# MingruiYuan/SpoofSV

Measured on AMD Instinct MI355X. Metric: mel-frames/sec (Text2Mel+SSRN train), higher is better.
Workload: dtype f32 (conv GEMMs: fp32 operands scaled by a power of two and split into fp16 hi+lo = 22 significand bits, three exact fp16 MFMAs per product, fp32 accumulate: ~2^-22 per product, gradients within 3e-6 of float64 = the exact-fp32 path's level); 1 GPU; train_text2mel + train_ssrn (train/ordinary.py step: fwd, l1+bin-div+guided-att losses, bwd, Adam), batch 32 utterances/GPU, N=186, T=325, 80 mel -> 513x1300 linear, hidden 256, random-init; global_batch=32, parallelism=dp1, launch=hipGraph replay, ddp=none

## Files before the change

### spoofsv_amd/csrc/api.hip

```cpp
#include <stdarg.h>
#include <stdio.h>
#include <stdlib.h>
#include <string.h>
#include "ssv_common.h"

static thread_local char g_err[512] = "";
int ssv_fail(int code, const char* fmt, ...) {
  va_list ap;
  va_start(ap, fmt);
  vsnprintf(g_err, sizeof(g_err), fmt, ap);
  va_end(ap);
  return code;
}
int ssv_check_launch(const char* what) {
  hipError_t e = hipGetLastError();
  if (e == hipSuccess) return 0;
  ssv_fail(0, "%s: launch failed: %s", what, hipGetErrorString(e));
  return -(int)e;
}
static int g_precision = -1;
static int precision_from_env() {
  const char* e = getenv("SSV_PRECISION");
  if (!e || !*e || !strcmp(e, "f16x2") || !strcmp(e, "2")) return 2;
  if (!strcmp(e, "fp32") || !strcmp(e, "0")) return 0;
  if (!strcmp(e, "bf16x3") || !strcmp(e, "1")) return 1;
  return -1;
}
int ssv_precision() {
  if (g_precision < 0) {
    g_precision = precision_from_env();
    if (g_precision < 0) {
      fprintf(stderr, "libssv_hip: SSV_PRECISION=%s is not one of fp32|0, bf16x3|1, f16x2|2 (call ssv_set_precision to choose a mode)\n", getenv("SSV_PRECISION"));
      abort();
    }
  }
  return g_precision;
}
static const char* const g_knob_names[SSV_T_COUNT] = {"SSV_NT_FORCE", "SSV_NNB_FORCE", "SSV_LN_GROUPS", "SSV_LN_PERSIST", "SSV_LSTM_MERGE", "SSV_PWLN_BWD"};
static char g_knob_val[SSV_T_COUNT][512];
static const char* g_knob[SSV_T_COUNT];
static int g_knobs_loaded = 0;
static void load_knobs() {
  for (int i = 0; i < SSV_T_COUNT; ++i) {
    const char* e = getenv(g_knob_names[i]);
    if (e) { strncpy(g_knob_val[i], e, sizeof g_knob_val[i] - 1); g_knob_val[i][sizeof g_knob_val[i] - 1] = 0; g_knob[i] = g_knob_val[i]; }
    else g_knob[i] = nullptr;
  }
  __atomic_store_n(&g_knobs_loaded, 1, __ATOMIC_RELEASE);
}
const char* ssv_tuning(int knob) {
  if (!__atomic_load_n(&g_knobs_loaded, __ATOMIC_ACQUIRE)) load_knobs();
  return g_knob[knob];
}
extern "C" void ssv_reload_tuning(void) { load_knobs(); }
#include <mutex>
#include <string>
#include <map>
static int g_shape_log = -1;
static std::string g_shape_path;
static std::mutex g_shape_mu;
static std::map<std::string, long>* g_shape_seen = nullptr;
static void shape_log_flush() {
  std::lock_guard<std::mutex> lk(g_shape_mu);
  if (!g_shape_seen) return;
  if (g_shape_path.empty()) return;
  if (FILE* f = fopen(g_shape_path.c_str(), "w")) {
    for (const auto& kv : *g_shape_seen) fprintf(f, "%s\t%ld\n", kv.first.c_str(), kv.second);
    fclose(f);
  }
}
bool ssv_shape_log_on() {
  if (g_shape_log < 0) { const char* e = getenv("SSV_SHAPE_LOG"); g_shape_log = (e && *e) ? 1 : 0; if (g_shape_log) { g_shape_path = e; atexit(shape_log_flush); } }
  return g_shape_log == 1;
}
void ssv_shape_log(const char* kernel, dim3 grid, dim3 block, double flops, double bytes, const char* note) {
  if (!ssv_shape_log_on()) return;
  char line[768];
  snprintf(line, sizeof line, "%s\t%ux%ux%u\t%.6g\t%.6g\t%s", kernel, grid.x * block.x, grid.y * block.y, grid.z * block.z, flops, bytes, note ? note : "");
  std::lock_guard<std::mutex> lk(g_shape_mu);
  if (!g_shape_seen) g_shape_seen = new std::map<std::string, long>();
  ++(*g_shape_seen)[line];
}
extern "C" int ssv_set_precision(int mode) {
  int prev = g_precision >= 0 ? g_precision : precision_from_env();
  if (prev < 0) prev = ssv_fail(SSV_UNSUPPORTED, "SSV_PRECISION=%s is not one of fp32|0, bf16x3|1, f16x2|2; mode %d set explicitly", getenv("SSV_PRECISION"), mode);
  g_precision = mode <= 0 ? 0 : (mode == 1 ? 1 : 2);
  return prev;
}
extern "C" int ssv_get_precision(void) {
  if (g_precision < 0 && precision_from_env() < 0)
    return ssv_fail(SSV_UNSUPPORTED, "SSV_PRECISION=%s is not one of fp32|0, bf16x3|1, f16x2|2", getenv("SSV_PRECISION"));
  return ssv_precision();
}
extern "C" int ssv_version(void) { return 7; }
extern "C" const char* ssv_arch(void) { return "gfx950"; }
extern "C" const char* ssv_last_error(void) { return g_err; }
```

### spoofsv_amd/csrc/api_norm.hip

```cpp
#include "ssv_host.h"

extern "C" size_t ssv_channel_ln_act_fwd_workspace(int B, int C, int L) { (void)B; (void)C; (void)L; return 256; }
extern "C" int ssv_channel_ln_act_fwd(const float* x, long x_bs, const float* gamma, const float* beta, float* y, long y_bs, float* y_amax, float* stats,
                                      int B, int C, int L, int act, void* ws, size_t ws_bytes, ssv_stream_t stream) {
  SSV_CHECK(x && gamma && beta && y && B > 0 && C > 0 && L > 0 && act >= 0 && act <= 2, SSV_BAD_SHAPE, "channel_ln_act_fwd: bad argument");
  SSV_CHECK(B <= 65535, SSV_UNSUPPORTED, "channel_ln_act_fwd: batch %d exceeds grid.y", B);
  (void)ws; (void)ws_bytes;
  return ssv_launch_ln_act_fwd(x, x_bs, gamma, beta, y, y_bs, stats, B, C, L, act, (hipStream_t)stream, y_amax);
}
static size_t ln_part_bytes(int B, int C, int L, int rows_per_block) { return align256((size_t)ssv_ln_gate_bwd_nblk(B, L) * rows_per_block * C * sizeof(float)); }
extern "C" size_t ssv_channel_ln_act_bwd_workspace(int B, int C, int L) { return ln_part_bytes(B, C, L, 3); }
extern "C" int ssv_channel_ln_act_bwd(const float* dy, long dy_bs, const float* x, long x_bs, const float* stats, const float* gamma, const float* beta,
                                      float* dx, long dx_bs, float* pgrads, int B, int C, int L, int act, void* ws, size_t ws_bytes, ssv_stream_t stream) {
  SSV_CHECK(dy && x && stats && gamma && beta && dx && B > 0 && C > 0 && L > 0 && act >= 0 && act <= 2, SSV_BAD_SHAPE, "channel_ln_act_bwd: bad argument");
  SSV_CHECK(ws && ws_bytes >= ssv_channel_ln_act_bwd_workspace(B, C, L), SSV_BAD_SHAPE, "channel_ln_act_bwd: workspace too small");
  return ssv_launch_ln_act_bwd(dy, dy_bs, x, x_bs, stats, gamma, beta, dx, dx_bs, (float*)ws, pgrads, B, C, L, act, (hipStream_t)stream);
}

static bool pwln_fused(int B, int Cin, int Cout, int L) { return use_bf3(B, L, Cin, Cout) && Cout <= 640 && B <= 65535; }
extern "C" size_t ssv_pointwise_conv_ln_act_fwd_workspace(int Cin, int Cout) { return conv_fwd_ws(Cin, Cout, 1).total; }
extern "C" int ssv_pointwise_conv_ln_act_fwd(const float* x, long x_bs, const float* x_amax, int x_namax, const float* w, const void* w_packed, const float* bias,
                                             const float* s, const float* gamma, const float* beta, float* pre, float* stats, float* y, long y_bs, float* y_amax,
                                             int B, int Cin, int Cout, int L, int act, void* ws, size_t ws_bytes, ssv_stream_t stream) {
  SSV_CHECK(x && w && gamma && beta && pre && y && B > 0 && Cin > 0 && Cout > 0 && L > 0 && act >= 0 && act <= 2, SSV_BAD_SHAPE, "pointwise_conv_ln_act_fwd: bad argument");
  SSV_CHECK(x_bs >= (long)Cin * L && y_bs >= (long)Cout * L, SSV_BAD_SHAPE, "pointwise_conv_ln_act_fwd: batch stride smaller than C*L");
  if (pwln_fused(B, Cin, Cout, L) && y_bs == (long)Cout * L && (!y_amax || ssv_amax_rows_(L) >= ssv_cdiv(L, 64))) {
    const ConvWs l = conv_fwd_ws(Cin, Cout, 1);
    SSV_CHECK((w_packed && !(use_f16() && !x_amax)) || (ws && ws_bytes >= l.total), SSV_BAD_SHAPE, "pointwise_conv_ln_act_fwd: workspace too small");
    int shift[3] = {0, 0, 0};
    PwLnArgs pw = {gamma, beta, y, y_bs, stats, y_amax, ssv_amax_rows_(L), act};
    return conv_nn(x, x_bs, w, packed_planes(w_packed, Cout, Cin, 1).fwd, (long)Cin, 1, bias, s, nullptr, 0, pre, (long)Cout * L, B, Cin, Cout, L, 1, shift, true,
                   ws, l, (hipStream_t)stream, x_amax, x_namax, nullptr, &pw);
  }
  SSV_TRY(ssv_conv1d_fwd(x, x_bs, x_amax, x_namax, w, w_packed, bias, s, pre, (long)Cout * L, nullptr, B, Cin, Cout, L, 1, 1, 0, ws, ws_bytes, stream));
  return ssv_channel_ln_act_fwd(pre, (long)Cout * L, gamma, beta, y, y_bs, y_amax, stats, B, Cout, L, act, nullptr, 0, stream);
}

static inline bool hw_colstats(int B, int C, int L) { return use_bf3(B, L, C, 2 * C) && C % 64 == 0 && C <= 512; }
struct HwFwdWs { ConvWs conv; size_t colstats, total; };
static HwFwdWs hw_fwd_ws(int B, int C, int L, int k) {
  HwFwdWs l;
  l.conv = conv_fwd_ws(C, 2 * C, k);
  WsTake t;
  t.take(l.conv.total);
  l.colstats = t.take(hw_colstats(B, C, L) ? (size_t)B * (2 * C / 64) * L * 2 * sizeof(float) : 0);
  l.total = t.off;
  return l;
}
extern "C" size_t ssv_highway_conv1d_fwd_workspace(int B, int C, int L, int k) { return hw_fwd_ws(B, C, L, k).total; }
extern "C" int ssv_highway_conv1d_fwd(const float* x, long x_bs, const float* x_amax, int x_namax, const float* w, const void* w_packed, const float* bias,
                                      const float* g1, const float* b1, const float* g2, const float* b2, float* h, float* stats, float* y, long y_bs,
                                      float* y_amax, int B, int C, int L, int k, int dilation, int causal, void* ws, size_t ws_bytes, ssv_stream_t stream) {
  SSV_CHECK(x && w && g1 && b1 && g2 && b2 && h && y, SSV_BAD_SHAPE, "highway_conv1d_fwd: null argument");
  SSV_CHECK(B > 0 && C > 0 && L > 0 && B <= 65535, SSV_BAD_SHAPE, "highway_conv1d_fwd: bad shape B=%d C=%d L=%d", B, C, L);
  if (hw_colstats(B, C, L)) {
    const HwFwdWs l = hw_fwd_ws(B, C, L, k);
    SSV_CHECK(ws && ws_bytes >= l.total, SSV_BAD_SHAPE, "highway_conv1d_fwd: workspace too small");
    SSV_CHECK(x_bs >= (long)C * L && y_bs >= (long)C * L, SSV_BAD_SHAPE, "highway_conv1d_fwd: batch stride smaller than C*L");
    float* cs = ws_f32(ws, l.colstats);
    int shift[3];
    SSV_TRY(conv_shifts(k, dilation, causal, shift));
    SSV_TRY(conv_nn(x, x_bs, w, packed_planes(w_packed, 2 * C, C, k).fwd, (long)C * k, k, bias, nullptr, nullptr, 0, h, (long)2 * C * L, B, C, 2 * C, L, k, shift, true,
                    ws, l.conv, (hipStream_t)stream, x_amax, x_namax, cs));
    return ssv_launch_ln_gate_fwd_stream(h, x, x_bs, cs, g1, b1, g2, b2, y, y_bs, stats, y_amax, B, C, L, (hipStream_t)stream);
  }
  SSV_TRY(ssv_conv1d_fwd(x, x_bs, x_amax, x_namax, w, w_packed, bias, nullptr, h, (long)2 * C * L, nullptr, B, C, 2 * C, L, k, dilation, causal, ws, ws_bytes, stream));
  return ssv_launch_ln_gate_fwd(h, (long)2 * C * L, x, x_bs, g1, b1, g2, b2, y, y_bs, stats, B, C, L, (hipStream_t)stream, y_amax);
}

static int pw_bwd_ln_and_data(const float* dy, long dy_bs, const float* w, const void* w_packed, const float* gamma, const float* beta, const float* pre,
                              const float* stats, float* dx, long dx_bs, float* dpre, float* dpre_amax, float* part, int B, int Cin, int Cout, int L, int act,
                              void* ws, size_t ws_bytes, ssv_stream_t stream) {
  const long pbs = (long)Cout * L;
  if (dx && w_packed && use_bf3(B, L, Cout, Cin) && (!use_f16() || dpre_amax) && ssv_pwln_bwd_fused_ok(B, Cin, Cout, L)) {
    const bool has_amax = dpre_amax != nullptr;
    const SplitPlanes pl = packed_planes(w_packed, Cout, Cin, 1).tr;
    PwLnBw q;
    q.dy = dy; q.dy_bs = dy_bs; q.pre = pre; q.stats = stats; q.gamma = gamma; q.beta = beta;
    q.dpre = dpre; q.part = part; q.part_rows = ssv_ln_act_bwd_rows(1, Cout, L, has_amax); q.part_q = 4 / ssv_ln_act_bwd_vec(Cout, L, has_amax);
    q.amax = dpre_amax; q.namax = ssv_amax_rows_(L);
    q.Ahi = pl.hi; q.Alo = pl.lo; q.a_inv = pl.inv;
    q.dx = dx; q.dx_bs = dx_bs;
    q.xrow_w = (Cin > 128 && Cin % 128 == 1) ? w + (Cin - 1) : nullptr; q.xrow_sk = Cin;
    q.M = Cout; q.Cin = Cin; q.L = L; q.act = act;
    return ssv_launch_pwln_bwd(q, B, use_f16() ? 1 : 0, (hipStream_t)stream);
  }
  SSV_TRY(ssv_launch_ln_act_bwd(dy, dy_bs, pre, pbs, stats, gamma, beta, dpre, pbs, part, nullptr, B, Cout, L, act, (hipStream_t)stream, dpre_amax));
  if (dx) SSV_TRY(ssv_conv1d_bwd_data(dpre, pbs, dpre_amax, ssv_amax_rows_(L), w, w_packed, nullptr, dx, dx_bs, B, Cin, Cout, L, 1, 1, 0, ws, ws_bytes, stream));
  return 0;
}
struct LinkBwdWs { size_t dpre, part, amax, data, data_bytes, wgrad, wgrad_bytes, total; };
static LinkBwdWs link_bwd_ws(int B, int Cin, int Cout, int L, int k) {
  WsTake t;
  LinkBwdWs l;
  l.dpre = t.take((size_t)B * Cout * L * sizeof(float));
  l.part = t.take(ln_part_bytes(B, Cout, L, 3));
  l.amax = t.take((size_t)B * ssv_amax_rows_(L) * sizeof(float));
  l.data_bytes = ssv_conv1d_bwd_data_workspace(Cin, Cout, k);
  l.data = t.take(l.data_bytes);
  l.wgrad_bytes = ssv_conv1d_bwd_weight_workspace(B, Cin, Cout, L, k);
  l.wgrad = t.take(l.wgrad_bytes);
  l.total = t.off;
  return l;
}
static LinkBwdWs pw_ws(int B, int Cin, int Cout, int L) { return link_bwd_ws(B, Cin, Cout, L, 1); }
static LinkBwdWs hw_ws(int B, int C, int L, int k) { return link_bwd_ws(B, C, 2 * C, L, k); }
extern "C" size_t ssv_pointwise_conv_ln_act_bwd_workspace(int B, int Cin, int Cout, int L) { return pw_ws(B, Cin, Cout, L).total; }
extern "C" int ssv_pointwise_conv_ln_act_bwd(const float* dy, long dy_bs, const float* x, long x_bs, const float* x_amax, int x_namax, const float* w,
                                             const void* w_packed, const float* gamma,
                                             const float* beta, const float* pre, const float* stats, float* dx, long dx_bs, float* dw, float* pgrads,
                                             float* ds, int B, int Cin, int Cout, int L, int act, void* ws, size_t ws_bytes, ssv_stream_t stream) {
  SSV_CHECK(dy && x && w && gamma && beta && pre && stats && dw && pgrads, SSV_BAD_SHAPE, "pointwise_conv_ln_act_bwd: null argument");
  SSV_CHECK(B > 0 && B <= 65535 && Cin > 0 && Cout > 0 && L > 0 && act >= 0 && act <= 2, SSV_BAD_SHAPE, "pointwise_conv_ln_act_bwd: bad shape");
  const LinkBwdWs s = pw_ws(B, Cin, Cout, L);
  SSV_CHECK(ws && ws_bytes >= s.total, SSV_BAD_SHAPE, "pointwise_conv_ln_act_bwd: workspace too small (%zu < %zu)", ws_bytes, s.total);
  float* dpre = ws_f32(ws, s.dpre);
  const long pbs = (long)Cout * L;
  float* da = use_f16() ? ws_f32(ws, s.amax) : nullptr;
  const int dn = ssv_amax_rows_(L);
  SSV_TRY(pw_bwd_ln_and_data(dy, dy_bs, w, w_packed, gamma, beta, pre, stats, dx, dx_bs, dpre, da, ws_f32(ws, s.part), B, Cin, Cout, L, act,
                             ws_f32(ws, s.data), s.data_bytes, stream));
  if (ds) SSV_TRY(ssv_rowsum(dpre, pbs, ds, B, Cout, L, stream));
  return conv1d_bwd_weight_impl(dpre, pbs, x, x_bs, dw, B, Cin, Cout, L, 1, 1, 0, ws_f32(ws, s.wgrad), s.wgrad_bytes, stream,
                                ws_f32(ws, s.part), pgrads, 3 * Cout, ssv_ln_act_bwd_rows(B, Cout, L, da != nullptr), da, dn, x_amax, x_namax);
}

extern "C" size_t ssv_channel_ln_bwd2_workspace(int B, int C, int L) { return ln_part_bytes(B, C, L, 1); }
extern "C" int ssv_channel_ln_bwd2(const float* v, long v_bs, const float* gn, long gn_bs, const float* x, long x_bs, const float* stats,
                                   const float* gamma, float* d_gn, long dgn_bs, float* d_x, long dx_bs, float* dgamma,
                                   int B, int C, int L, void* ws, size_t ws_bytes, ssv_stream_t stream) {
  SSV_CHECK(v && gn && x && stats && gamma && d_gn && d_x && dgamma && B > 0 && B <= 65535 && C > 0 && L > 0, SSV_BAD_SHAPE, "channel_ln_bwd2: bad argument");
  SSV_CHECK(ws && ws_bytes >= ssv_channel_ln_bwd2_workspace(B, C, L), SSV_BAD_SHAPE, "channel_ln_bwd2: workspace too small");
  return ssv_launch_ln_bwd2(v, v_bs, gn, gn_bs, x, x_bs, stats, gamma, d_gn, dgn_bs, d_x, dx_bs, (float*)ws, dgamma, B, C, L, (hipStream_t)stream);
}
extern "C" int ssv_highway_gate_fwd(const float* h, const float* x, long x_bs, const float* g1, const float* b1, const float* g2, const float* b2,
                                    float* stats, float* y, long y_bs, float* y_amax, int B, int C, int L, ssv_stream_t stream) {
  SSV_CHECK(h && x && g1 && b1 && g2 && b2 && y && B > 0 && B <= 65535 && C > 0 && L > 0, SSV_BAD_SHAPE, "highway_gate_fwd: bad argument");
  return ssv_launch_ln_gate_fwd(h, (long)2 * C * L, x, x_bs, g1, b1, g2, b2, y, y_bs, stats, B, C, L, (hipStream_t)stream, y_amax);
}
extern "C" size_t ssv_highway_gate_bwd2_workspace(int B, int C, int L) { return ln_part_bytes(B, C, L, 4); }
extern "C" int ssv_highway_gate_bwd2(const float* vh, const float* vx, long vx_bs, const float* gy, long gy_bs, const float* h, const float* x, long x_bs,
                                     const float* stats, const float* g1, const float* b1, const float* g2, const float* b2,
                                     float* d_gy, long dgy_bs, float* d_h, float* d_x, long dx_bs, float* pgrads,
                                     int B, int C, int L, void* ws, size_t ws_bytes, ssv_stream_t stream) {
  SSV_CHECK(vh && vx && gy && h && x && stats && g1 && b1 && g2 && b2 && d_gy && d_h && d_x && pgrads && B > 0 && B <= 65535 && C > 0 && L > 0,
            SSV_BAD_SHAPE, "highway_gate_bwd2: bad argument");
  SSV_CHECK(ws && ws_bytes >= ssv_highway_gate_bwd2_workspace(B, C, L), SSV_BAD_SHAPE, "highway_gate_bwd2: workspace too small");
  return ssv_launch_ln_gate_bwd2(vh, vx, vx_bs, gy, gy_bs, h, x, x_bs, stats, g1, b1, g2, b2, d_gy, dgy_bs, d_h, d_x, dx_bs, (float*)ws, pgrads,
                                 B, C, L, (hipStream_t)stream);
}

extern "C" size_t ssv_highway_gate_bwd_workspace(int B, int C, int L) { return ln_part_bytes(B, C, L, 6); }
extern "C" int ssv_highway_gate_bwd(const float* dy, long dy_bs, const float* x, long x_bs, const float* g1, const float* b1,
                                    const float* g2, const float* b2, const float* h, const float* stats, float* dh, float* dxres,
                                    long dx_bs, float* pgrads, int B, int C, int L, void* ws, size_t ws_bytes, ssv_stream_t stream) {
  SSV_CHECK(dy && x && g1 && b1 && g2 && b2 && h && stats && dh && dxres && B > 0 && C > 0 && L > 0 && B <= 65535, SSV_BAD_SHAPE, "highway_gate_bwd: bad argument");
  SSV_CHECK(ws && ws_bytes >= ssv_highway_gate_bwd_workspace(B, C, L), SSV_BAD_SHAPE, "highway_gate_bwd: workspace too small");
  return ssv_launch_ln_gate_bwd(dy, dy_bs, h, x, x_bs, stats, g1, b1, g2, b2, dh, dxres, dx_bs, (float*)ws, pgrads, B, C, L, (hipStream_t)stream);
}

extern "C" size_t ssv_highway_conv1d_bwd_workspace(int B, int C, int L, int k) { return hw_ws(B, C, L, k).total; }
extern "C" int ssv_highway_conv1d_bwd(const float* dy, long dy_bs, const float* x, long x_bs, const float* x_amax, int x_namax, const float* w, const void* w_packed,
                                      const float* g1, const float* b1,
                                      const float* g2, const float* b2, const float* h, const float* stats, float* dx, long dx_bs, float* dw,
                                      float* pgrads, int B, int C, int L, int k, int dilation, int causal, void* ws, size_t ws_bytes,
                                      ssv_stream_t stream) {
  SSV_CHECK(dy && x && w && g1 && b1 && g2 && b2 && h && stats && dx && dw && pgrads, SSV_BAD_SHAPE, "highway_conv1d_bwd: null argument");
  SSV_CHECK(B > 0 && C > 0 && L > 0 && B <= 65535, SSV_BAD_SHAPE, "highway_conv1d_bwd: bad shape B=%d C=%d L=%d", B, C, L);
  const LinkBwdWs s = hw_ws(B, C, L, k);
  SSV_CHECK(ws && ws_bytes >= s.total, SSV_BAD_SHAPE, "highway_conv1d_bwd: workspace too small (%zu < %zu)", ws_bytes, s.total);
  float* dH = ws_f32(ws, s.dpre);
  float* da = use_f16() ? ws_f32(ws, s.amax) : nullptr;
  const int dn = ssv_amax_rows_(L);
  SSV_TRY(ssv_launch_ln_gate_bwd(dy, dy_bs, h, x, x_bs, stats, g1, b1, g2, b2, dH, dx, dx_bs, ws_f32(ws, s.part), nullptr, B, C, L, (hipStream_t)stream, da));
  SSV_TRY(ssv_conv1d_bwd_data(dH, (long)2 * C * L, da, dn, w, w_packed, dx, dx, dx_bs, B, C, 2 * C, L, k, dilation, causal, ws_f32(ws, s.data), s.data_bytes, stream));
  return conv1d_bwd_weight_impl(dH, (long)2 * C * L, x, x_bs, dw, B, C, 2 * C, L, k, dilation, causal, ws_f32(ws, s.wgrad), s.wgrad_bytes, stream,
                                ws_f32(ws, s.part), pgrads, 6 * C, ssv_ln_gate_bwd_rows(B, C, L, da != nullptr), da, dn, x_amax, x_namax);
}

extern "C" int ssv_ln_partial_rows(int B, int L) { return ssv_ln_gate_bwd_nblk(B, L); }
extern "C" int ssv_ln_bwd_partial_rows(int gate, int B, int C, int L, int with_amax) {
  return gate ? ssv_ln_gate_bwd_rows(B, C, L, with_amax != 0) : ssv_ln_act_bwd_rows(B, C, L, with_amax != 0);
}
extern "C" size_t ssv_highway_conv1d_bwd_data_workspace(int B, int C, int L, int k) { (void)B; (void)L; return ssv_conv1d_bwd_data_workspace(C, 2 * C, k); }
extern "C" int ssv_highway_conv1d_bwd_data(const float* dy, long dy_bs, const float* x, long x_bs, const float* w, const void* w_packed,
                                           const float* g1, const float* b1, const float* g2, const float* b2, const float* h, const float* stats,
                                           float* dx, long dx_bs, float* dh, float* dh_amax, float* part, int B, int C, int L, int k, int dilation, int causal,
                                           void* ws, size_t ws_bytes, ssv_stream_t stream) {
  SSV_CHECK(dy && x && w && g1 && b1 && g2 && b2 && h && stats && dx && dh && part, SSV_BAD_SHAPE, "highway_conv1d_bwd_data: null argument");
  SSV_CHECK(B > 0 && C > 0 && L > 0 && B <= 65535, SSV_BAD_SHAPE, "highway_conv1d_bwd_data: bad shape B=%d C=%d L=%d", B, C, L);
  SSV_TRY(ssv_launch_ln_gate_bwd(dy, dy_bs, h, x, x_bs, stats, g1, b1, g2, b2, dh, dx, dx_bs, part, nullptr, B, C, L, (hipStream_t)stream, dh_amax));
  return ssv_conv1d_bwd_data(dh, (long)2 * C * L, dh_amax, ssv_amax_rows_(L), w, w_packed, dx, dx, dx_bs, B, C, 2 * C, L, k, dilation, causal, ws, ws_bytes, stream);
}
extern "C" size_t ssv_pointwise_conv_ln_act_bwd_data_workspace(int B, int Cin, int Cout, int L) { (void)B; (void)L; return ssv_conv1d_bwd_data_workspace(Cin, Cout, 1); }
extern "C" int ssv_pointwise_conv_ln_act_bwd_data(const float* dy, long dy_bs, const float* w, const void* w_packed, const float* gamma, const float* beta,
                                                  const float* pre, const float* stats, float* dx, long dx_bs, float* ds, float* dpre, float* dpre_amax,
                                                  float* part, int B, int Cin, int Cout, int L, int act, void* ws, size_t ws_bytes, ssv_stream_t stream) {
  SSV_CHECK(dy && w && gamma && beta && pre && stats && dpre && part, SSV_BAD_SHAPE, "pointwise_conv_ln_act_bwd_data: null argument");
  SSV_CHECK(B > 0 && B <= 65535 && Cin > 0 && Cout > 0 && L > 0 && act >= 0 && act <= 2, SSV_BAD_SHAPE, "pointwise_conv_ln_act_bwd_data: bad shape");
  const long pbs = (long)Cout * L;
  SSV_TRY(pw_bwd_ln_and_data(dy, dy_bs, w, w_packed, gamma, beta, pre, stats, dx, dx_bs, dpre, dpre_amax, part, B, Cin, Cout, L, act, ws, ws_bytes, stream));
  if (ds) SSV_TRY(ssv_rowsum(dpre, pbs, ds, B, Cout, L, stream));
  return 0;
}
```

### spoofsv_amd/csrc/bf3_tuning.h

```cpp
#pragma once

#ifndef SSV_NN_XONE
#define SSV_NN_XONE 1
#endif

#define SSV_NN_XBUF(KT, WM, NT) (!((KT) == 3 && (NT) == 6))

#ifndef SSV_NN_HALO_SMALL
#define SSV_NN_HALO_SMALL 16
#endif

#define SSV_NNB_WAVES(KT, WM, NT, EPI, HW) \
  (((KT) == 1 && (WM) == 2 && (NT) == 4 && (EPI) == 0) || ((KT) == 3 && (WM) == 2 && (NT) == 7 && (EPI) == 0 && (HW) == 16) ? 3 : 2)

#ifndef SSV_NNBW_XROW
#define SSV_NNBW_XROW 1
#endif

#ifndef SSV_NNBW_PARK
#define SSV_NNBW_PARK 1
#endif

#ifndef SSV_NT_RING
#define SSV_NT_RING 1
#endif

#ifndef SSV_NT_XROW
#define SSV_NT_XROW 1
#endif

#ifndef SSV_PWLN_XROW
#define SSV_PWLN_XROW 1
#endif

#ifndef SSV_PWLN_ROLL
#define SSV_PWLN_ROLL 1
#endif

#ifndef SSV_PWLN_PARK
#define SSV_PWLN_PARK 1
#endif

#ifndef SSV_PWLN_BWD_FUSED
#define SSV_PWLN_BWD_FUSED 1
#endif
#ifndef SSV_PWLN_BK64
#define SSV_PWLN_BK64 1
#endif
#ifndef SSV_NT3R_ABL
#define SSV_NT3R_ABL 0
#endif
#ifndef SSV_LSTM_FAST_CELL
#define SSV_LSTM_FAST_CELL 1
#endif
#ifndef SSV_NT_NOBREAK
#define SSV_NT_NOBREAK 1
#endif
#ifndef SSV_NT_SPLIT_FIRST
#define SSV_NT_SPLIT_FIRST 1
#endif
#ifndef SSV_LSTM_PRESPLIT
#define SSV_LSTM_PRESPLIT 1
#endif
#ifndef SSV_LSTM_ABL
#define SSV_LSTM_ABL 0
#endif
#ifndef SSV_LSTM_X0FOLD
#define SSV_LSTM_X0FOLD 1
#endif
#ifndef SSV_LSTM_PRESPLIT_TRAIN
#define SSV_LSTM_PRESPLIT_TRAIN 1
#endif
```

### spoofsv_amd/csrc/ssv_common.h

```cpp
#pragma once
#include <hip/hip_runtime.h>
#include <stdint.h>
#include <stddef.h>
#include "../../include/ssv_hip.h"

int ssv_fail(int code, const char* fmt, ...);
#define SSV_BAD_SHAPE (-1)
#define SSV_UNSUPPORTED (-2)
#define SSV_CHECK(cond, code, ...) do { if (!(cond)) return ssv_fail((code), __VA_ARGS__); } while (0)
#define SSV_TRY(expr) do { int _e = (expr); if (_e) return _e; } while (0)
int ssv_check_launch(const char* what);

typedef __attribute__((ext_vector_type(4))) float f32x4;

struct GemmNN {
  const float* A = nullptr; long sab = 0, sam = 0, sac = 0, saj = 0;
  const float* X = nullptr; long sxb = 0, sxc = 0, sxn = 1; int Lx = 0;
  float* C = nullptr; long scb = 0, scm = 0, scn = 1;
  const float* bias = nullptr;
  const float* bias_b = nullptr; long sbb = 0;
  const float* R = nullptr; long srb = 0, srm = 0, srn = 1;
  int M = 0, N = 0, Kc = 0, KT = 1, B = 1;
  int shift[3] = {0, 0, 0};
  float alpha = 1.f;
};
int ssv_launch_gemm_nn(const GemmNN& g, hipStream_t st);

struct GemmNT {
  const float* A = nullptr; long sab = 0, sam = 0, sat = 1; int La = 0;
  const float* X = nullptr; long sxb = 0, sxc = 0, sxn = 1; int Lx = 0;
  float* C = nullptr; long scz = 0, scm = 0, scc = 1, scj = 0;
  int M = 0, Nc = 0, KT = 1, B = 1, Z = 1, bstep = 1;
  int shift[3] = {0, 0, 0};
  const ssv_wgrad_job* jobs = nullptr; int njobs = 0;
  int max_shift = -1;
  int f16 = 0; const float* a_amax = nullptr; int a_namax = 0; const float* x_amax = nullptr; int x_namax = 0;
};
int ssv_launch_gemm_nt(const GemmNT& g, hipStream_t st);

struct GemmNNB {
  const unsigned short* Ahi = nullptr; const unsigned short* Alo = nullptr; int Kpad = 0;
  const float* X = nullptr; long sxb = 0, sxc = 0; int Lx = 0;
  float* C = nullptr; long scb = 0, scm = 0;
  const float* bias = nullptr;
  const float* bias_b = nullptr; long sbb = 0;
  const float* R = nullptr; long srb = 0, srm = 0;
  int M = 0, N = 0, Kc = 0, KT = 1, B = 1;
  int shift[3] = {0, 0, 0};
  int sxn = 1, scn = 1;
  int row_pair = 0; float* c_amax = nullptr; int c_namax = 0;
  unsigned short* hs_planes = nullptr; long hs_plane_bytes = 0; int hs_npad = 0;
  int hs_keep_h = 1;
  int ksplit = 1; long scz = 0; int skip_rows = 0;
  const unsigned short* x0_planes = nullptr; const float* x0_amax = nullptr; int xsplit0 = 0;
  int perm_h = 0, epi = 0, first = 0;
  float* cstate = nullptr;
  float* lstm_out = nullptr; int lstm_s = 0, lstm_lo = 0, lstm_D = 0, xsplit = 0; long sab = 0;
  const unsigned short* A0hi = nullptr; const unsigned short* A0lo = nullptr;
  float* gates_out = nullptr;
  int f16 = 0; const float* a_inv = nullptr; const float* x_amax = nullptr; int x_namax = 0; long x_amax_bs = 0;
  float* colstats = nullptr;
  const float* xrow_w = nullptr; long xrow_sk = 0;
};
int ssv_launch_gemm_nn_bf3(const GemmNNB& g, hipStream_t st);
int ssv_launch_gemm_pwln(const GemmNNB& g, const float* gamma, const float* beta, float* y, long ybs, float* stats, float* y_amax, int namax, int act,
                         hipStream_t st);
int ssv_launch_gemm_nt_bf3(const GemmNT& g, hipStream_t st);
int ssv_launch_gemm_nt3r(const GemmNT& g, dim3 grid, int mtiles, int tchunks, int ring_ms, hipStream_t st);
struct PwLnBw {
  const float* dy; long dy_bs; const float* pre; const float* stats; const float* gamma; const float* beta;
  float* dpre; float* part; int part_rows; int part_q; float* amax; int namax;
  const unsigned short* Ahi; const unsigned short* Alo; const float* a_inv;
  float* dx; long dx_bs; const float* xrow_w; long xrow_sk;
  int M, Cin, L, act;
};
bool ssv_pwln_bwd_fused_ok(int B, int Cin, int Cout, int L);
int ssv_launch_pwln_bwd(const PwLnBw& q, int B, int f16, hipStream_t st);
bool ssv_nt_bf3_xrow(int KT, int M, int Nc);
bool ssv_nt_bf3_fits(const GemmNT& g);
int ssv_launch_pack_split(const float* w, void* hi, void* lo, int M, int K, int Kpad, int KT, long sm, long sk, long sj, int perm_h, hipStream_t st,
                          int nch_total = 0, int ch_off = 0);
int ssv_launch_pack_split_f16(const float* w, long w_elems, void* hi, void* lo, int M, int K, int Kpad, int KT, long sm, long sk, long sj, float* aux, hipStream_t st);
int ssv_launch_pack_split_f16_list(const float* w, void* hi, void* lo, int M, int K, int Kpad, int KT, long sm, long sk, long sj, int perm_h,
                                   const float* list, int nlist, float* inv_out, hipStream_t st, int nch_total = 0, int ch_off = 0);
#define SSV_F16_AUX_FLOATS 128
#define SSV_AMAX_FALLBACK 64
int ssv_launch_absmax(const float* x, long x_bs, int B, long n, float* out, int npb, hipStream_t st);
int ssv_nt_bf3_tiles(int KT, int M, int Nc);
void ssv_nt_bf3_tile(int KT, int M, int Nc, int* wm, int* ntc);
int ssv_nt_bf3_wg_per_cu(int KT, int wm, int ntc);
int ssv_precision();
enum { SSV_T_NT_FORCE, SSV_T_NNB_FORCE, SSV_T_LN_GROUPS, SSV_T_LN_PERSIST, SSV_T_LSTM_MERGE, SSV_T_PWLN_BWD, SSV_T_COUNT };
const char* ssv_tuning(int knob);
int ssv_pack_job_blocks(const ssv_pack_job& j);
int ssv_launch_pack_multi(const ssv_pack_job* jobs_dev, int njobs, int nblocks, float* amax_ws, hipStream_t st);
#define SSV_PACK_AMAX_PER_WEIGHT 32

int ssv_launch_reduce_slabs(const float* slabs, float* out, long n, int Z, long slab_stride, hipStream_t st);
int ssv_launch_reduce_slabs_perm(const float* slabs, float* out, int M, int Nc, int KT, int Z, hipStream_t st);
int ssv_launch_reduce_pair(const float* slabs, float* out, int M, int Nc, int KT, int Z, const float* part, float* pout, int n2, int nblk, hipStream_t st);
int ssv_launch_reduce_pair_multi(const ssv_wgrad_job* jobs, int njobs, const float* slabs, int M, int Nc, int KT, int Z, int n2, int nblk, hipStream_t st);
int ssv_launch_pack_wt(const float* w, float* wt, int Cout, int Cin, int KT, hipStream_t st);
int ssv_launch_fill(float* p, float v, long n, hipStream_t st);
int ssv_launch_linear_len1_fwd(const float* x, long x_bs, const float* w, const float* bias, const float* bias_b, long sbb, float* y, long y_bs,
                               int B, int K, int M, hipStream_t st);
int ssv_launch_linear_len1_wgrad(const float* dy, long dy_bs, const float* x, long x_bs, float* dw, int B, int K, int M, hipStream_t st);

static inline int ssv_cdiv(long a, long b) { return (int)((a + b - 1) / b); }
bool ssv_shape_log_on();
void ssv_shape_log(const char* kernel, dim3 grid, dim3 block, double flops, double bytes, const char* note);
__host__ __device__ static inline int ssv_amax_rows_(int L) { return 4 * ((L + 63) / 64); }

__device__ __forceinline__ unsigned ssv_xcd_order(unsigned lin, unsigned total) {
  const unsigned xcd = lin & 7u, idx = lin >> 3, q = total >> 3, r = total & 7u;
  return xcd * q + (xcd < r ? xcd : r) + idx;
}

__device__ __forceinline__ void ssv_pow2_scale(float amax, float& scale, float& inv) {
  int E = (int)((__float_as_uint(amax) >> 23) & 0xffu);
  E = min(max(E, 15), 254);
  scale = __uint_as_float((unsigned)(268 - E) << 23);
  inv = __uint_as_float((unsigned)(E - 14) << 23);
}
typedef unsigned ssv_u32x4g __attribute__((vector_size(16)));
__device__ __forceinline__ __amdgpu_buffer_rsrc_t ssv_buf(const void* base) {
  return __builtin_amdgcn_make_buffer_rsrc(const_cast<void*>(base), 0, -1, 0x00020000);
}
__device__ __forceinline__ float ssv_buf_f32(__amdgpu_buffer_rsrc_t r, unsigned voff, unsigned soff) {
  return __builtin_bit_cast(float, __builtin_amdgcn_raw_buffer_load_b32(r, (int)voff, (int)soff, 0));
}
__device__ __forceinline__ uint4 ssv_buf_u4(__amdgpu_buffer_rsrc_t r, unsigned voff, unsigned soff) {
  return __builtin_bit_cast(uint4, __builtin_amdgcn_raw_buffer_load_b128(r, (int)voff, (int)soff, 0));
}
template <class T> __device__ __forceinline__ T* ssv_global(T* p) {
  return (T*)(__attribute__((address_space(1))) T*)p;
}
__device__ __forceinline__ float ssv_uniform(float v) { return __builtin_bit_cast(float, __builtin_amdgcn_readfirstlane(__builtin_bit_cast(int, v))); }
template <int NW>
__device__ __forceinline__ float ssv_wg_max(float v, float* sm) {
#pragma unroll
  for (int o = 1; o < 64; o <<= 1) v = fmaxf(v, __shfl_xor(v, o));
  if ((threadIdx.x & 63) == 0) sm[threadIdx.x >> 6] = v;
  __syncthreads();
  float r = sm[0];
#pragma unroll
  for (int i = 1; i < NW; ++i) r = fmaxf(r, sm[i]);
  return r;
}
template <int CTRL> __device__ __forceinline__ float ssv_dpp_mov(float v);
template <int CTRL>
__device__ __forceinline__ float ssv_dpp_max(float v) { return fmaxf(v, ssv_dpp_mov<CTRL>(v)); }
__device__ __forceinline__ float ssv_wave_list_max(const float* __restrict__ p, int n) {
  float v = 0.f;
  for (int i = threadIdx.x & 63; i < n; i += 64) v = fmaxf(v, p[i]);
  v = ssv_dpp_max<0xB1>(v);
  v = ssv_dpp_max<0x4E>(v);
  v = ssv_dpp_max<0x141>(v);
  v = ssv_dpp_max<0x140>(v);
  const int b = __builtin_bit_cast(int, v);
  const float r0 = __builtin_bit_cast(float, __builtin_amdgcn_readlane(b, 0)), r1 = __builtin_bit_cast(float, __builtin_amdgcn_readlane(b, 16));
  const float r2 = __builtin_bit_cast(float, __builtin_amdgcn_readlane(b, 32)), r3 = __builtin_bit_cast(float, __builtin_amdgcn_readlane(b, 48));
  return fmaxf(fmaxf(r0, r1), fmaxf(r2, r3));
}
template <int NW>
__device__ __forceinline__ float ssv_list_max(const float* __restrict__ p, int n, float* sm) {
  float v = 0.f;
  for (int i = threadIdx.x; i < n; i += 64 * NW) v = fmaxf(v, p[i]);
  return ssv_wg_max<NW>(v, sm);
}

template <int CTRL>
__device__ __forceinline__ float ssv_dpp_mov(float v) {
  return __builtin_bit_cast(float, __builtin_amdgcn_update_dpp(0, __builtin_bit_cast(int, v), CTRL, 0xf, 0xf, true));
}
__device__ __forceinline__ float ssv_row16_sum(float v) {
  v += ssv_dpp_mov<0xB1>(v);
  v += ssv_dpp_mov<0x4E>(v);
  v += ssv_dpp_mov<0x141>(v);
  v += ssv_dpp_mov<0x140>(v);
  return v;
}
__device__ __forceinline__ float ssv_wave_sum(float v) {
  v = ssv_row16_sum(v);
  v += __shfl_xor(v, 16);
  v += __shfl_xor(v, 32);
  return v;
}
```

Baseline: 913,500 mel-frames/s.

## Fuse highway conv1d forward GEMM with dual layernorm and gate into one kernel

Adds a single kernel for the C=256, k=3 highway conv forward path. It computes the split-precision conv GEMM, the bias, two channel layernorms, the sigmoid gate and the residual mix in one pass, and writes h, stats, y and the y amax directly. This removes the separate column-stats pass and the normalisation/gate kernels, along with the HBM round trip of the pre-activation. By default it is enabled only for L in {325, 1300}, with an env knob to override. Risks are register and LDS pressure from the large kernel and reduced occupancy compared with the tuned standalone GEMM.

Result: no change. 921,000 mel-frames/s (median of 6 runs) (+0.8%).

```diff
diff --git a/spoofsv_amd/csrc/api.hip b/spoofsv_amd/csrc/api.hip
--- a/spoofsv_amd/csrc/api.hip
+++ b/spoofsv_amd/csrc/api.hip
@@ -36,7 +36,7 @@
   }
   return g_precision;
 }
-static const char* const g_knob_names[SSV_T_COUNT] = {"SSV_NT_FORCE", "SSV_NNB_FORCE", "SSV_LN_GROUPS", "SSV_LN_PERSIST", "SSV_LSTM_MERGE", "SSV_PWLN_BWD"};
+static const char* const g_knob_names[SSV_T_COUNT] = {"SSV_NT_FORCE", "SSV_NNB_FORCE", "SSV_LN_GROUPS", "SSV_LN_PERSIST", "SSV_LSTM_MERGE", "SSV_PWLN_BWD", "SSV_HWY_FUSED"};
 static char g_knob_val[SSV_T_COUNT][512];
 static const char* g_knob[SSV_T_COUNT];
 static int g_knobs_loaded = 0;
diff --git a/spoofsv_amd/csrc/api_norm.hip b/spoofsv_amd/csrc/api_norm.hip
--- a/spoofsv_amd/csrc/api_norm.hip
+++ b/spoofsv_amd/csrc/api_norm.hip
@@ -53,6 +53,29 @@
                                       float* y_amax, int B, int C, int L, int k, int dilation, int causal, void* ws, size_t ws_bytes, ssv_stream_t stream) {
   SSV_CHECK(x && w && g1 && b1 && g2 && b2 && h && y, SSV_BAD_SHAPE, "highway_conv1d_fwd: null argument");
   SSV_CHECK(B > 0 && C > 0 && L > 0 && B <= 65535, SSV_BAD_SHAPE, "highway_conv1d_fwd: bad shape B=%d C=%d L=%d", B, C, L);
+  if (w_packed && ssv_precision() >= 1 && C == 256 && k == 3 && ssv_highway_fused_wanted(B, L)) {
+    int shift[3];
+    SSV_TRY(conv_shifts(k, dilation, causal, shift));
+    if (ssv_highway_fused_shape_ok(B, C, L, k, shift)) {
+      SSV_CHECK(x_bs >= (long)C * L && y_bs >= (long)C * L, SSV_BAD_SHAPE, "highway_conv1d_fwd: batch stride smaller than C*L");
+      const HwFwdWs l = hw_fwd_ws(B, C, L, k);
+      const SplitPlanes pl = packed_planes(w_packed, 2 * C, C, k).fwd;
+      HwFused q = {};
+      q.Ahi = pl.hi; q.Alo = pl.lo; q.a_inv = pl.inv;
+      q.x = x; q.x_bs = x_bs;
+      if (use_f16()) {
+        SSV_CHECK(x_amax || (ws && ws_bytes >= l.total), SSV_BAD_SHAPE, "highway_conv1d_fwd: workspace too small");
+        AmaxList xa;
+        SSV_TRY(amax_of(x, x_bs, B, (long)C * L, x_amax, x_namax, ws ? ws_f32(ws, l.conv.fb) : nullptr, &xa, (hipStream_t)stream));
+        q.x_amax = xa.p; q.x_namax = xa.n;
+      }
+      q.bias = bias; q.g1 = g1; q.b1 = b1; q.g2 = g2; q.b2 = b2;
+      q.h = h; q.stats = stats; q.y = y; q.y_bs = y_bs; q.y_amax = y_amax;
+      q.L = L;
+      for (int j = 0; j < 3; ++j) q.shift[j] = shift[j];
+      return ssv_launch_highway_fused(q, B, use_f16() ? 1 : 0, (hipStream_t)stream);
+    }
+  }
   if (hw_colstats(B, C, L)) {
     const HwFwdWs l = hw_fwd_ws(B, C, L, k);
     SSV_CHECK(ws && ws_bytes >= l.total, SSV_BAD_SHAPE, "highway_conv1d_fwd: workspace too small");
diff --git a/spoofsv_amd/csrc/bf3_tuning.h b/spoofsv_amd/csrc/bf3_tuning.h
--- a/spoofsv_amd/csrc/bf3_tuning.h
+++ b/spoofsv_amd/csrc/bf3_tuning.h
@@ -44,6 +44,15 @@
 #ifndef SSV_PWLN_BWD_FUSED
 #define SSV_PWLN_BWD_FUSED 1
 #endif
+#ifndef SSV_HWY_FUSED_LENGTHS
+#define SSV_HWY_FUSED_LENGTHS {325, 1300}
+#endif
+#ifndef SSV_HWF_NT
+#define SSV_HWF_NT 4
+#endif
+#ifndef SSV_HWF_WARM
+#define SSV_HWF_WARM 1
+#endif
 #ifndef SSV_PWLN_BK64
 #define SSV_PWLN_BK64 1
 #endif
diff --git a/spoofsv_amd/csrc/highway_fused.hip b/spoofsv_amd/csrc/highway_fused.hip
--- /dev/null
+++ b/spoofsv_amd/csrc/highway_fused.hip
@@ -0,0 +1,312 @@
+#include "bf3_common.h"
+
+#ifdef SSV_HWF_STAMP
+__device__ unsigned long long ssv_hwf_stamps[1024 * 8];
+extern "C" int ssv_debug_hwf_stamps(unsigned long long* out) { return (int)hipMemcpyFromSymbol(out, HIP_SYMBOL(ssv_hwf_stamps), sizeof(ssv_hwf_stamps)); }
+#define HWF_STAMP(k) do { const unsigned w_ = blockIdx.y * gridDim.x + blockIdx.x; if (threadIdx.x == 0 && w_ < 1024u) \
+    ssv_hwf_stamps[w_ * 8 + (k)] = ((k) >= 6) ? __builtin_amdgcn_s_memrealtime() : __builtin_readcyclecounter(); } while (0)
+__device__ unsigned long long ssv_hwf_launch[64 * 4];
+extern "C" int ssv_debug_hwf_launches(unsigned long long* out) { return (int)hipMemcpyFromSymbol(out, HIP_SYMBOL(ssv_hwf_launch), sizeof(ssv_hwf_launch)); }
+#define HWF_LAUNCH(slot, which) do { if (threadIdx.x == 0) { \
+    if (blockIdx.x == 0 && blockIdx.y == 0) ssv_hwf_launch[(slot) * 4 + (which)] = __builtin_amdgcn_s_memrealtime(); \
+    if (blockIdx.x == gridDim.x - 1 && blockIdx.y == gridDim.y - 1) ssv_hwf_launch[(slot) * 4 + 2 + (which)] = __builtin_amdgcn_s_memrealtime(); } } while (0)
+#else
+#define HWF_STAMP(k) do {} while (0)
+#define HWF_LAUNCH(slot, which) do {} while (0)
+#endif
+template <int F16, int HW>
+__global__ __launch_bounds__(512, 2) void highway_fused_kernel(const HwFused q) {
+  constexpr int C = 256, NCH = C / 32, MB = 2 * C / 16, NT = SSV_HWF_NT, BN = 16 * NT;
+  constexpr int WX = ((BN + HW + 15) / 16) * 16;
+  constexpr int X_SLOTS = 4 * WX;
+  static_assert(X_SLOTS <= 512, "one slot per thread");
+  constexpr int IMG = 2 * X_SLOTS;
+  constexpr unsigned APLANE_B = (unsigned)MB * NCH * 1024u;
+  constexpr int LDWP = BN + 4;
+  __shared__ uint4 lds[2][IMG];
+  __shared__ float park[8 * 16 * LDWP];
+  __shared__ float red[8][2][BN];
+  __shared__ float colv[4][BN];
+  __shared__ float amx[8];
+  const int tid = threadIdx.x, lane = tid & 63, wave = tid >> 6;
+  const unsigned wg = ssv_xcd_order(blockIdx.x + gridDim.x * blockIdx.y, gridDim.x * gridDim.y);
+  const int ntile = (int)(wg % gridDim.x), b = (int)(wg / gridDim.x);
+  const int n0 = ntile * BN, L = q.L;
+  const int kq = lane >> 4, nq = lane & 15;
+  const float* __restrict__ Xb = q.x + (long)b * q.x_bs;
+#ifdef SSV_HWF_STAMP
+  const int span = q.span & 0xffff, slot = (q.span >> 16) & 63;
+#else
+  const int span = q.span;
+#endif
+  HWF_STAMP(6); HWF_STAMP(0); HWF_LAUNCH(slot, 0);
+
+  f32x4 acc[4][NT];
+#pragma unroll
+  for (int i = 0; i < 4; ++i)
+#pragma unroll
+    for (int t = 0; t < NT; ++t) acc[i][t] = (f32x4){0.f, 0.f, 0.f, 0.f};
+  unsigned arowb[4];
+#pragma unroll
+  for (int i = 0; i < 4; ++i) arowb[i] = (unsigned)((((i >> 1) * (MB / 2) + wave * 2 + (i & 1)) * NCH * 512 + lane * 8) * 2);
+  const __amdgpu_buffer_rsrc_t rsAh = ssv_buf(q.Ahi), rsAl = ssv_buf(q.Alo);
+  uint4 Ah_[4], Al_[4];
+  const __amdgpu_buffer_rsrc_t rsX = __builtin_amdgcn_make_buffer_rsrc(const_cast<float*>(Xb), 0, (int)(((long)(C - 1) * L + L) * 4), 0x00020000);
+  const bool stager = tid < X_SLOTS;
+  const int skg = stager ? tid / WX : 0, scol = tid % WX;
+  const int gcol = n0 + q.smin + scol;
+  const bool cvs = stager && scol < BN + span && gcol >= 0 && gcol < L;
+  const unsigned voffb = (unsigned)(8 * skg * L + min(max(gcol, 0), L - 1)) * 4u;
+  float rx[8];
+  auto prefetchX = [&](int ch) __attribute__((always_inline)) {
+#pragma unroll
+    for (int i = 0; i < 8; ++i) rx[i] = ssv_buf_f32(rsX, voffb, (unsigned)((ch * 32 + i) * L) * 4u);
+  };
+  float xs = 1.f, xinv = 1.f, ainv = 1.f;
+  if constexpr (F16) ainv = *q.a_inv;
+  auto commitX = [&](int ch) __attribute__((always_inline)) {
+    if (!stager) return;
+    float v[8];
+#pragma unroll
+    for (int i = 0; i < 8; ++i) v[i] = cvs ? rx[i] : 0.f;
+    uint4 h, l;
+    split8s<F16>(v, xs, h, l);
+    lds[ch & 1][tid] = h; lds[ch & 1][X_SLOTS + tid] = l;
+  };
+  int offj[3];
+#pragma unroll
+  for (int j = 0; j < 3; ++j) offj[j] = q.shift[j] - q.smin;
+  uint4 fh[2][NT], fl[2][NT];
+  auto frags = [&](int ch, int j, uint4 (&h)[NT], uint4 (&l)[NT]) __attribute__((always_inline)) {
+    const uint4* Xh = lds[ch & 1];
+    const uint4* Xl = lds[ch & 1] + X_SLOTS;
+#pragma unroll
+    for (int t = 0; t < NT; ++t) { const int s_ = kq * WX + t * 16 + nq + offj[j]; h[t] = Xh[s_]; l[t] = Xl[s_]; }
+  };
+
+#pragma unroll
+  for (int i = 0; i < 4; ++i) { Ah_[i] = ssv_buf_u4(rsAh, arowb[i], 0u); Al_[i] = ssv_buf_u4(rsAl, arowb[i], 0u); }
+  prefetchX(0);
+  if constexpr (F16) {
+    float sc, inv;
+    ssv_pow2_scale(ssv_wave_list_max(q.x_amax + (long)b * q.x_namax, q.x_namax), sc, inv);
+    xs = ssv_uniform(sc); xinv = ssv_uniform(inv);
+  }
+  commitX(0);
+  prefetchX(1);
+  unsigned warm = 0u;
+  if constexpr (SSV_HWF_WARM) {
+    const unsigned unit = (unsigned)__builtin_amdgcn_readfirstlane((int)(((blockIdx.x + gridDim.x * blockIdx.y) >> 3) % 24u));
+    warm = __builtin_amdgcn_raw_buffer_load_b32(unit < 12u ? rsAh : rsAl, (int)(((unit % 12u) * 512u + (unsigned)tid) * 128u), 0, 0);
+  }
+  __syncthreads();
+  HWF_STAMP(1);
+  for (int ch = 0; ch < NCH; ++ch) {
+    frags(ch, 0, fh[0], fl[0]);
+#pragma unroll
+    for (int j = 0; j < 3; ++j) {
+      const unsigned ubn = (unsigned)__builtin_amdgcn_readfirstlane((int)(j < 2 ? (unsigned)(j + 1) * APLANE_B + (unsigned)ch * 1024u
+                                                                                  : (unsigned)min(ch + 1, NCH - 1) * 1024u));
+#pragma unroll
+      for (int i = 0; i < 4; ++i) {
+        if (i == 0 && j < 2) frags(ch, j + 1, fh[(j + 1) & 1], fl[(j + 1) & 1]);
+        __builtin_amdgcn_sched_barrier(0);
+#pragma unroll
+        for (int t = 0; t < NT; ++t) {
+          acc[i][t] = mma16<F16>(Al_[i], fh[j & 1][t], acc[i][t]);
+          acc[i][t] = mma16<F16>(Ah_[i], fl[j & 1][t], acc[i][t]);
+          acc[i][t] = mma16<F16>(Ah_[i], fh[j & 1][t], acc[i][t]);
+        }
+        __builtin_amdgcn_sched_barrier(0);
+        Ah_[i] = ssv_buf_u4(rsAh, arowb[i], ubn);
+        Al_[i] = ssv_buf_u4(rsAl, arowb[i], ubn);
+        if (j == 1 && i == 1) commitX(ch + 1);
+        if (j == 1 && i == 2) prefetchX(min(ch + 2, NCH - 1));
+        __builtin_amdgcn_sched_barrier(0);
+      }
+    }
+    __syncthreads();
+  }
+
+  HWF_STAMP(2);
+  if constexpr (SSV_HWF_WARM) asm volatile("" :: "v"(warm));
+  const float us = F16 ? ssv_uniform(xinv * ainv) : 1.f;
+  float* __restrict__ Hb = q.h + (long)b * 2 * C * L;
+  float* __restrict__ Yb = q.y + (long)b * q.y_bs;
+  float* pk = park + wave * 16 * LDWP;
+  auto store_block = [&](float* __restrict__ dst, int rbase) __attribute__((always_inline)) {
+#pragma unroll
+    for (int it = 0; it < NT; ++it) {
+      const int e = lane + 64 * it;
+      const int row = e / (BN / 4), c4 = e % (BN / 4);
+      const int gn = n0 + c4 * 4;
+      const f32x4 v = *reinterpret_cast<const f32x4*>(pk + row * LDWP + c4 * 4);
+      if (gn < L) {
+        float* o = dst + (long)(rbase + row) * L + gn;
+        if (gn + 3 < L) { f4u w = {v[0], v[1], v[2], v[3]}; *reinterpret_cast<f4u*>(o) = w; }
+        else {
+#pragma unroll
+          for (int j = 0; j < 4; ++j) if (gn + j < L) o[j] = v[j];
+        }
+      }
+    }
+  };
+  float addv[4][4], ga1[2][4], be1[2][4], ga2[2][4], be2[2][4], xres[2][4][NT];
+#pragma unroll
+  for (int i = 0; i < 4; ++i)
+#pragma unroll
+    for (int r = 0; r < 4; ++r) addv[i][r] = q.bias ? q.bias[(i >> 1) * C + (wave * 2 + (i & 1)) * 16 + kq * 4 + r] : 0.f;
+#pragma unroll
+  for (int i = 0; i < 2; ++i)
+#pragma unroll
+    for (int r = 0; r < 4; ++r) {
+      const int c = (wave * 2 + i) * 16 + kq * 4 + r;
+      ga1[i][r] = q.g1[c]; be1[i][r] = q.b1[c]; ga2[i][r] = q.g2[c]; be2[i][r] = q.b2[c];
+#pragma unroll
+      for (int t = 0; t < NT; ++t) xres[i][r][t] = ssv_buf_f32(rsX, (unsigned)(c * L + min(n0 + t * 16 + nq, L - 1)) * 4u, 0u);
+    }
+  float s1[NT], s2[NT];
+#pragma unroll
+  for (int t = 0; t < NT; ++t) s1[t] = s2[t] = 0.f;
+#pragma unroll
+  for (int i = 0; i < 4; ++i) {
+#pragma unroll
+    for (int r = 0; r < 4; ++r) {
+      const float add = addv[i][r];
+#pragma unroll
+      for (int t = 0; t < NT; ++t) {
+        const float v = (F16 ? acc[i][t][r] * us : acc[i][t][r]) + add;
+        acc[i][t][r] = v;
+        if (i < 2) s1[t] += v; else s2[t] += v;
+        pk[(kq * 4 + r) * LDWP + t * 16 + nq] = v;
+      }
+    }
+    store_block(Hb, (i >> 1) * C + (wave * 2 + (i & 1)) * 16);
+  }
+  auto col_reduce = [&](float (&u)[NT], float (&v)[NT], int slot) __attribute__((always_inline)) {
+#pragma unroll
+    for (int t = 0; t < NT; ++t) {
+      u[t] += __shfl_xor(u[t], 16); u[t] += __shfl_xor(u[t], 32);
+      v[t] += __shfl_xor(v[t], 16); v[t] += __shfl_xor(v[t], 32);
+    }
+    if (kq == 0) {
+#pragma unroll
+      for (int t = 0; t < NT; ++t) { red[wave][0][t * 16 + nq] = u[t]; red[wave][1][t * 16 + nq] = v[t]; }
+    }
+    __syncthreads();
+    if (tid < 2 * BN) {
+      const int half = tid / BN, col = tid % BN;
+      float s_ = 0.f;
+#pragma unroll
+      for (int w = 0; w < 8; ++w) s_ += red[w][half][col];
+      colv[2 * slot + half][col] = s_;
+    }
+    __syncthreads();
+  };
+  col_reduce(s1, s2, 0);
+  HWF_STAMP(3);
+  const float invC = 1.f / (float)C;
+  float mu1[NT], mu2[NT], q1[NT], q2[NT];
+#pragma unroll
+  for (int t = 0; t < NT; ++t) { mu1[t] = colv[0][t * 16 + nq] * invC; mu2[t] = colv[1][t * 16 + nq] * invC; q1[t] = q2[t] = 0.f; }
+#pragma unroll
+  for (int i = 0; i < 2; ++i)
+#pragma unroll
+    for (int r = 0; r < 4; ++r)
+#pragma unroll
+      for (int t = 0; t < NT; ++t) {
+        const float d1 = acc[i][t][r] - mu1[t], d2 = acc[2 + i][t][r] - mu2[t];
+        q1[t] += d1 * d1; q2[t] += d2 * d2;
+      }
+  col_reduce(q1, q2, 1);
+  HWF_STAMP(4);
+  float r1[NT], r2[NT];
+#pragma unroll
+  for (int t = 0; t < NT; ++t) { r1[t] = rsqrtf(colv[2][t * 16 + nq] * invC + 1e-5f); r2[t] = rsqrtf(colv[3][t * 16 + nq] * invC + 1e-5f); }
+  if (q.stats && wave == 0 && kq == 0) {
+#pragma unroll
+    for (int t = 0; t < NT; ++t) {
+      const int gn = n0 + t * 16 + nq;
+      if (gn < L) { float* sb = q.stats + (long)b * 4 * L + gn; sb[0] = mu1[t]; sb[L] = r1[t]; sb[2L * L] = mu2[t]; sb[3L * L] = r2[t]; }
+    }
+  }
+  float am = 0.f;
+#pragma unroll
+  for (int i = 0; i < 2; ++i) {
+#pragma unroll
+    for (int r = 0; r < 4; ++r)
+#pragma unroll
+      for (int t = 0; t < NT; ++t) {
+        const float n1 = (acc[i][t][r] - mu1[t]) * r1[t] * ga1[i][r] + be1[i][r];
+        const float n2 = (acc[2 + i][t][r] - mu2[t]) * r2[t] * ga2[i][r] + be2[i][r];
+        const float s = __builtin_amdgcn_rcpf(1.f + __expf(-n1));
+        const float yv = s * n2 + (1.f - s) * xres[i][r][t];
+        if (n0 + t * 16 + nq < L) am = fmaxf(am, fabsf(yv));
+        pk[(kq * 4 + r) * LDWP + t * 16 + nq] = yv;
+      }
+    store_block(Yb, (wave * 2 + i) * 16);
+  }
+  HWF_STAMP(5); HWF_STAMP(7); HWF_LAUNCH(slot, 1);
+  if (q.y_amax) {
+#pragma unroll
+    for (int o = 1; o < 64; o <<= 1) am = fmaxf(am, __shfl_xor(am, o));
+    if (lane == 0) amx[wave] = am;
+    __syncthreads();
+    float* al = q.y_amax + (long)b * q.namax;
+    if constexpr (NT == 4) {
+      if (tid < 4) al[4 * ntile + tid] = fmaxf(amx[2 * tid], amx[2 * tid + 1]);
+    } else if (tid == 0) {
+      float m = amx[0];
+#pragma unroll
+      for (int w = 1; w < 8; ++w) m = fmaxf(m, amx[w]);
+      al[ntile] = m;
+      if (ntile == (int)gridDim.x - 1) for (int e = gridDim.x; e < q.namax; ++e) al[e] = 0.f;
+    }
+  }
+}
+
+bool ssv_highway_fused_shape_ok(int B, int C, int L, int k, const int* shift) {
+  if (C != 256 || k != 3 || B > 65535 || L < 1 || (long)2 * C * L >= (1L << 29)) return false;
+  int smin = shift[0], smax = shift[0];
+  for (int j = 1; j < 3; ++j) { smin = shift[j] < smin ? shift[j] : smin; smax = shift[j] > smax ? shift[j] : smax; }
+  return smax - smin <= 54;
+}
+bool ssv_highway_fused_wanted(int B, int L) {
+  int mode = 1;
+  if (const char* e = ssv_tuning(SSV_T_HWY_FUSED)) mode = atoi(e);
+  if (mode == 0) return false;
+  if (mode == 2) return true;
+  if ((long)B * L < 128) return false;
+  static const int table[] = SSV_HWY_FUSED_LENGTHS;
+  for (int l : table) if (l == L) return true;
+  return false;
+}
+int ssv_launch_highway_fused(HwFused q, int B, int f16, hipStream_t st) {
+  SSV_CHECK(ssv_highway_fused_shape_ok(B, 256, q.L, 3, q.shift), SSV_UNSUPPORTED, "highway_fused: shape not supported (L=%d)", q.L);
+  SSV_CHECK(q.Ahi && q.Alo && q.x && q.g1 && q.b1 && q.g2 && q.b2 && q.h && q.y, SSV_BAD_SHAPE, "highway_fused: null argument");
+  SSV_CHECK(!f16 || (q.a_inv && q.x_amax && q.x_namax > 0), SSV_BAD_SHAPE, "highway_fused: split-fp16 needs operand scales");
+  int smin = q.shift[0], smax = q.shift[0];
+  for (int j = 1; j < 3; ++j) { smin = q.shift[j] < smin ? q.shift[j] : smin; smax = q.shift[j] > smax ? q.shift[j] : smax; }
+  q.smin = smin; q.span = smax - smin;
+  const dim3 grid(ssv_cdiv(q.L, 16 * SSV_HWF_NT), B);
+  q.namax = ssv_amax_rows_(q.L);
+  const bool small = SSV_NN_HALO_SMALL >= 0 && q.span <= SSV_NN_HALO_SMALL && SSV_NN_HALO_SMALL <= 16;
+  if (ssv_shape_log_on()) {
+    char nm[96], note[96];
+    snprintf(nm, sizeof nm, "highway_fused_kernel<%d, %d>", f16, small ? 16 : 54);
+    snprintf(note, sizeof note, "B=%d C=256 L=%d k=3 span=%d conv + 2 LN + gate", B, q.L, q.span);
+    ssv_shape_log(nm, grid, dim3(512), 2.0 * B * 512 * q.L * 256 * 3, 4.0 * B * 256.0 * q.L * 5, note);
+  }
+#ifdef SSV_HWF_STAMP
+  static int launches = 0;
+  q.span |= (launches++ & 63) << 16;
+#endif
+  if (small) {
+    if (f16) hipLaunchKernelGGL((highway_fused_kernel<1, 16>), grid, dim3(512), 0, st, q);
+    else hipLaunchKernelGGL((highway_fused_kernel<0, 16>), grid, dim3(512), 0, st, q);
+  } else {
+    if (f16) hipLaunchKernelGGL((highway_fused_kernel<1, 54>), grid, dim3(512), 0, st, q);
+    else hipLaunchKernelGGL((highway_fused_kernel<0, 54>), grid, dim3(512), 0, st, q);
+  }
+  return ssv_check_launch("highway_fused");
+}
diff --git a/spoofsv_amd/csrc/ssv_common.h b/spoofsv_amd/csrc/ssv_common.h
--- a/spoofsv_amd/csrc/ssv_common.h
+++ b/spoofsv_amd/csrc/ssv_common.h
@@ -76,6 +76,16 @@
 };
 bool ssv_pwln_bwd_fused_ok(int B, int Cin, int Cout, int L);
 int ssv_launch_pwln_bwd(const PwLnBw& q, int B, int f16, hipStream_t st);
+struct HwFused {
+  const unsigned short* Ahi; const unsigned short* Alo; const float* a_inv;
+  const float* x; long x_bs; const float* x_amax; int x_namax;
+  const float* bias; const float* g1; const float* b1; const float* g2; const float* b2;
+  float* h; float* stats; float* y; long y_bs; float* y_amax; int namax;
+  int L; int shift[3]; int smin, span;
+};
+bool ssv_highway_fused_shape_ok(int B, int C, int L, int k, const int* shift);
+bool ssv_highway_fused_wanted(int B, int L);
+int ssv_launch_highway_fused(HwFused q, int B, int f16, hipStream_t st);
 bool ssv_nt_bf3_xrow(int KT, int M, int Nc);
 bool ssv_nt_bf3_fits(const GemmNT& g);
 int ssv_launch_pack_split(const float* w, void* hi, void* lo, int M, int K, int Kpad, int KT, long sm, long sk, long sj, int perm_h, hipStream_t st,
@@ -90,7 +100,7 @@
 void ssv_nt_bf3_tile(int KT, int M, int Nc, int* wm, int* ntc);
 int ssv_nt_bf3_wg_per_cu(int KT, int wm, int ntc);
 int ssv_precision();
-enum { SSV_T_NT_FORCE, SSV_T_NNB_FORCE, SSV_T_LN_GROUPS, SSV_T_LN_PERSIST, SSV_T_LSTM_MERGE, SSV_T_PWLN_BWD, SSV_T_COUNT };
+enum { SSV_T_NT_FORCE, SSV_T_NNB_FORCE, SSV_T_LN_GROUPS, SSV_T_LN_PERSIST, SSV_T_LSTM_MERGE, SSV_T_PWLN_BWD, SSV_T_HWY_FUSED, SSV_T_COUNT };
 const char* ssv_tuning(int knob);
 int ssv_pack_job_blocks(const ssv_pack_job& j);
 int ssv_launch_pack_multi(const ssv_pack_job* jobs_dev, int njobs, int nblocks, float* amax_ws, hipStream_t st);
```
